# matthiasverstraete/3d_recognizer

Measured on AMD Instinct MI355X. Metric: training clouds/sec, N=40960 pts, bs=8, at 1/2/4/8 GPUs; mIoU parity, higher is better.
Workload: dtype f32 storage/accumulate, bf16x3 MFMA in the wide GEMMs

## Files before the change

3d_recognizer_amd/csrc/rows.hip:

```cpp
#include "rl_common.h"

namespace {

struct RowsParams {
    const float* src;
    long lds, src_bstride;
    float* dst;
    long ldd;
    long rows, rows_per_batch;
    int C;
    const int32_t* i32;
    const int64_t* i64;
    int shared;
    int accumulate;
    RlLazy lazy;
};

template <typename I>
__device__ __forceinline__ long src_row(const RowsParams& p, I r) {
    const I b = r / (I)p.rows_per_batch;
    const I i = r - b * (I)p.rows_per_batch;
    long j = i;
    if (p.i32) j = p.shared ? p.i32[i] : p.i32[r];
    else if (p.i64) j = p.shared ? p.i64[i] : p.i64[r];
// ... 188 lines not shown
    }
}

template <typename I>
__global__ __launch_bounds__(256) void attpool_bwd_kernel(const float* __restrict__ X, const float* __restrict__ S,
                                                          const float* __restrict__ Pout, const float* __restrict__ dP,
                                                          long P, int K, int C, float* __restrict__ dS,
                                                          float* __restrict__ dXa) {
    const long total = P * C;
    for (long e = (long)blockIdx.x * 256 + threadIdx.x; e < total; e += (long)gridDim.x * 256) {
        const long pt = (long)((I)e / (I)C);
        const int c = (int)(e - pt * C);
        const long base = pt * K * C + c;
        float m = S[base];
        for (int k = 1; k < K; ++k) m = fmaxf(m, S[base + (long)k * C]);
        float den = 0.f;
        for (int k = 0; k < K; ++k) den += expf(S[base + (long)k * C] - m);
        const float inv = 1.f / den, g = dP[e], po = Pout[e];
        for (int k = 0; k < K; ++k) {
            const long o = base + (long)k * C;
            const float a = expf(S[o] - m) * inv;
            dXa[o] = g * a;
            dS[o] = a * g * (X[o] - po);
        }
    }
}

__global__ __launch_bounds__(256) void add_act_fwd_vec_kernel(const float* __restrict__ Y1, const float* __restrict__ s1,
                                                              const float* __restrict__ b1, const float* __restrict__ Y2,
                                                              const float* __restrict__ s2, const float* __restrict__ b2,
                                                              long quads, int C, float slope, float* __restrict__ O) {
    typedef float v4f __attribute__((ext_vector_type(4)));
    const unsigned cq = (unsigned)C >> 2;
    const long stride = (long)gridDim.x * 256;
    auto one = [&](long q) {
        const int c = (int)((unsigned long)q % cq) * 4;
        const v4f y1 = *reinterpret_cast<const v4f*>(Y1 + q * 4), y2 = *reinterpret_cast<const v4f*>(Y2 + q * 4);
        const v4f a1 = *reinterpret_cast<const v4f*>(s1 + c), c1 = *reinterpret_cast<const v4f*>(b1 + c);
        const v4f a2 = *reinterpret_cast<const v4f*>(s2 + c), c2 = *reinterpret_cast<const v4f*>(b2 + c);
        const v4f z = (y1 * a1 + c1) + (y2 * a2 + c2);
        v4f o;
#pragma unroll
        for (int j = 0; j < 4; ++j) o[j] = z[j] > 0.f ? z[j] : z[j] * slope;
        *reinterpret_cast<v4f*>(O + q * 4) = o;
    };
    long q = (long)blockIdx.x * 256 + threadIdx.x;
// ... 215 lines not shown
        hipLaunchKernelGGL(attpool_fwd_kernel<int64_t>, dim3(grid_for(P * C)), dim3(256), 0, (hipStream_t)stream, X, S, (long)P, K, C, Pout);
    }
    rl_note_kernel("attpool_fwd_kernel");
    RL_LAUNCH_CHECK("rl_attpool_fwd");
    return RL_OK;
}

extern "C" int rl_attpool_bwd(const float* X, const float* S, const float* Pout, const float* dP, int64_t P, int K,
                              int C, float* dS, float* dXa, void* stream) {
    RL_REQUIRE(X && S && Pout && dP && dS && dXa && P >= 0 && K > 0 && C > 0, RL_ERR_ARGS, "rl_attpool_bwd: bad arguments");
    if (P == 0) return RL_OK;
    if (fits32(P * C) && K == 16)
        hipLaunchKernelGGL(attpool_bwd16_kernel<uint32_t>, dim3(grid_for(P * C)), dim3(256), 0, (hipStream_t)stream, X, S, Pout, dP,
                           (long)P, C, dS, dXa);
    else if (fits32(P * C))
        hipLaunchKernelGGL(attpool_bwd_kernel<uint32_t>, dim3(grid_for(P * C)), dim3(256), 0, (hipStream_t)stream, X, S, Pout, dP,
                           (long)P, K, C, dS, dXa);
    else
        hipLaunchKernelGGL(attpool_bwd_kernel<int64_t>, dim3(grid_for(P * C)), dim3(256), 0, (hipStream_t)stream, X, S, Pout, dP,
                           (long)P, K, C, dS, dXa);
    rl_note_kernel("attpool_bwd_kernel");
    RL_LAUNCH_CHECK("rl_attpool_bwd");
    return RL_OK;
}

extern "C" int rl_add_act_fwd(const float* Y1, const float* s1, const float* b1, const float* Y2, const float* s2,
                              const float* b2, int64_t rows, int C, float slope, float* O, void* stream) {
    RL_REQUIRE(Y1 && s1 && b1 && Y2 && s2 && b2 && O && rows >= 0 && C > 0, RL_ERR_ARGS, "rl_add_act_fwd: bad arguments");
    if (rows == 0) return RL_OK;
    const bool vec = C % 4 == 0 && ((((uintptr_t)Y1) | ((uintptr_t)Y2) | ((uintptr_t)O) | ((uintptr_t)s1) | ((uintptr_t)b1) |
                                      ((uintptr_t)s2) | ((uintptr_t)b2)) & 15) == 0;
    if (vec) {
        const long quads = (long)rows * (C / 4);
        hipLaunchKernelGGL(add_act_fwd_vec_kernel, dim3(grid_for((quads + 1) / 2)), dim3(256), 0, (hipStream_t)stream, Y1, s1, b1, Y2,
                           s2, b2, quads, C, slope, O);
    } else if (fits32(rows * C))
        hipLaunchKernelGGL(add_act_fwd_kernel<uint32_t>, dim3(grid_for(rows * C)), dim3(256), 0, (hipStream_t)stream, Y1, s1, b1, Y2,
                           s2, b2, (long)rows * C, C, slope, O);
    else
        hipLaunchKernelGGL(add_act_fwd_kernel<int64_t>, dim3(grid_for(rows * C)), dim3(256), 0, (hipStream_t)stream, Y1, s1, b1, Y2,
                           s2, b2, (long)rows * C, C, slope, O);
    rl_note_kernel("add_act_fwd_kernel");
    RL_LAUNCH_CHECK("rl_add_act_fwd");
    return RL_OK;
}

// ... 130 lines not shown
```

3d_recognizer_amd/randlanet/_engine.py:

```python
from typing import Dict, List, Optional

import torch

from . import _hip as H
from . import _ops as ops
from ._ops import Lazy, Rpe

BN_EPS = 1e-6
BN_MOMENTUM = 0.99
BN_PIVOT = True
BAND_SORT_MIN_POINTS = 4096


class _Tape(list):

    def __init__(self):
        super().__init__()
        self.levels: List[int] = []

    def append(self, rec) -> None:
        super().append(rec)
        self.levels.append(ops.LEVEL)

    def clear(self) -> None:
# ... 127 lines not shown
            ctx.tape.append(("linear", a, out, wname, bname, ks, ns, True))
            outs.append(out)
        return outs[0], outs[1]

    def _mlp(self, ctx, a, name: str, n_out: int, act: int = H.ACT_NONE, slope: float = 0.0, *, transposed=False,
             bn=True, a_grad=True) -> Lazy:
        return self._linear(ctx, a, f"{name}.conv.weight", f"{name}.conv.bias", n_out, transposed=transposed,
                            bn=f"{name}.batch_norm" if bn else None, act=act, slope=slope, a_grad=a_grad)

    def _pool(self, ctx, name: str, u, g: Lazy, idx: torch.Tensor, csr, n: int, d: int, n_out: int, stage: int = 0,
              next_stats: bool = False) -> Lazy:
        B, K, h = u.B, self.K, d // 2
        rows = B * n * K
        Ws = self.P[f"{name}.score_fn.0.weight"]
        if ops.pool_supported(d, K):
            if next_stats:
                res, st2, ns2 = ops.pool_fwd(u, g, idx, Ws, n, d, stage, next_stats=True)
                ctx.next_stats = (st2, ns2)
            else:
                res = ops.pool_fwd(u, g, idx, Ws, n, d, stage)
            pooled = ops.plain(res, B, n)
            ctx.tape.append(("pool_fused", name, u, g, csr, idx, pooled, n, d, stage))
            return self._mlp(ctx, pooled, f"{name}.mlp", n_out, H.ACT_RELU)
        X = torch.empty((rows, d), dtype=torch.float32, device=u.raw.device)
        ops.copy_rows_pair(((u.raw, (0, h), n * K, X, (0, h), rows, n * K), dict(lazy=u)),
                           ((g.raw, (0, h), g.bstride, X, (h, h), rows, n * K), dict(index=idx, lazy=g)))
        S = ops.gemm(ops.plain(X, B, n * K), Ws, 1, d, d, None, wsplit=getattr(ctx, "wsplit", None))
        Pt = ops.attpool_fwd(X, S, B * n, K)
        pooled = ops.plain(Pt, B, n)
        ctx.tape.append(("pool", name, u, g, csr, X, S, pooled, n, d))
        return self._mlp(ctx, pooled, f"{name}.mlp", n_out, H.ACT_RELU)

    def _virtual_bn(self, ctx: Context, vr, stage: int, bn_name: str, stats=None, nslots: int = 1) -> Lazy:
        if ctx.training and stats is None:
            stats, nslots = ops.rpe_stats(vr, stage)
        scale, shift, mean, invstd = self._fold(ctx, bn_name, stats, vr.rows, vr.h, None, nslots)
        rec = Lazy(vr.d2, vr.B, vr.n * 16, vr.n * 16, vr.h, scale, shift, H.ACT_RELU, 0.0, mean, invstd, bn_name)
        return rec

    def _lfa(self, ctx, l: int, xin: Lazy, xyz: torch.Tensor, n: int, d: int, idx, d2, csr=None) -> Lazy:
        e = f"encoder.{l}"
        B, K, h = xin.B, self.K, d // 2
        ctx.keep += [idx, d2]
        ctx.bn_defer = [] if self.sync is None else None
        f0, sc = self._mlp_pair(ctx, xin, (f"{e}.mlp1", h, H.ACT_LRELU, 0.2), (f"{e}.shortcut", 2 * d, H.ACT_NONE, 0.0))
        if ops.virtual_rpe_supported(d, K, B * n, n):
# ... 4 lines not shown
            ops.bn_finalize_flush(ctx.bn_defer)
            q1 = self._pool(ctx, f"{e}.pool1", vr, f0, idx, csr, n, d, h, stage=1, next_stats=ctx.training)
            vr.bn2 = self._virtual_bn(ctx, vr, 2, f"{e}.mlp_rpe2.batch_norm", *getattr(ctx, "next_stats", (None, 1)))
            ctx.next_stats = (None, 1)
            ops.bn_finalize_flush(ctx.bn_defer)
            ctx.bn_defer = None
            q2 = self._pool(ctx, f"{e}.pool2", vr, q1, idx, csr, n, d, d, stage=2)
        else:
            rpe = Rpe(xyz, idx, d2, B, n, K)
            if h <= 128:
                rpe = ops.rpe_build(rpe)
            u1 = self._mlp(ctx, rpe, f"{e}.mlp_rpe1", h, H.ACT_RELU, a_grad=False)
            ops.bn_finalize_flush(ctx.bn_defer)
            q1 = self._pool(ctx, f"{e}.pool1", u1, f0, idx, csr, n, d, h)
            u2 = self._mlp(ctx, u1, f"{e}.mlp_rpe2", h, H.ACT_RELU)
            ops.bn_finalize_flush(ctx.bn_defer)
            ctx.bn_defer = None
            q2 = self._pool(ctx, f"{e}.pool2", u2, q1, idx, csr, n, d, d)
        m2 = self._mlp(ctx, q2, f"{e}.mlp2", 2 * d)
        O = ops.plain(ops.add_act_fwd(m2, sc, 0.01), B, n)
        ctx.tape.append(("add_act", m2, sc, O))
        return O

    def _wide_weight_uses(self, training: bool):
        uses = []
        for name, W in self.P.items():
            if not name.endswith(("conv.weight", "score_fn.0.weight")) or W.dim() < 2:
                continue
            a, b = int(W.shape[0]), int(W.shape[1])
            if max(a, b) <= 64:
                if name.endswith(".mlp1.conv.weight") and b % 32 == 0 and b > 64:
                    sc = self.P.get(name.replace(".mlp1.", ".shortcut."))
                    if sc is not None and int(sc.shape[0]) > 64:
                        uses.append((W.view(a, b), 1, b, b, a, True))
                continue
            transposed = name.startswith("decoder.")
            K, N = (a, b) if transposed else (b, a)
            ks, ns = (N, 1) if transposed else (1, K)
            W2 = W.view(a, b)
            uses.append((W2, ks, ns, K, N))
            if training:
                uses.append((W2, ns, ks, N, K))
        return uses

    def min_points(self) -> int:
        L = len(self.layers)
        return max(self.K * self.dec ** (L - 1), 2 * self.dec ** L)

    def prepare(self, inp: torch.Tensor, perm: torch.Tensor, training: bool) -> "Prep":
        B, N, cin = inp.shape
        assert cin == 3 + self.F and inp.dtype == torch.float32 and inp.is_cuda and inp.is_contiguous()
        assert perm.dtype == torch.int64 and perm.numel() == N and perm.is_cuda
# ... 36 lines not shown
        prep.xyz4, prep.searches = xyz4, searches
        prep.csrs = ops.csr_build([(searches[i][0], tasks[i][0]) for i in range(2 * L)]) if training else [None] * (2 * L)
        return prep

    def forward(self, inp: torch.Tensor, perm: torch.Tensor, training: bool, dropout_p: float = 0.5,
                keep_mask: Optional[torch.Tensor] = None, logits_out: Optional[torch.Tensor] = None,
                prep: Optional["Prep"] = None, head: Optional[ops.Head] = None):
        B, N, cin = inp.shape
        assert cin == 3 + self.F and inp.dtype == torch.float32 and inp.is_cuda and inp.is_contiguous()
        assert perm.dtype == torch.int64 and perm.numel() == N and perm.is_cuda
        assert N >= self.min_points()
        dev = inp.device
        ctx = Context()
        ctx.training, ctx.B, ctx.N, ctx.perm = training, B, N, perm
        L, dec = len(self.layers), self.dec
        ctx.eval_folds = None
        ctx.eval_sig = tuple(ops.virtual_rpe_supported(d, self.K, B * (N // dec ** l), N // dec ** l) for l, d in enumerate(self.layers))
        if not training:
            self._eval_spec_build = {}
            spec = self._eval_specs.get(ctx.eval_sig)
            if spec is not None and self.sync is None:
                ctx.eval_folds = self._eval_folds(spec)

        ctx.wsplit = ops.split_weights(self._wide_weight_uses(training))
        if prep is None:
            prep = self.prepare(inp, perm, training)
        perm = prep.perm
        ctx.perm = perm
        assert prep.B == B and prep.N == N and prep.training >= training
        inp_p, xyz, searches, csrs = prep.inp_p, prep.xyz, prep.searches, prep.csrs
        ctx.keep += [inp_p, xyz]
        if prep.xyz4 is not None:
            ctx.keep.append(prep.xyz4)
        ctx.xyz4 = prep.xyz4

        a0 = ops.plain(inp_p, B, N)
        if cin == 3 and prep.xyz4 is not None:
            a0 = Lazy(prep.xyz4.view(B * N, 4), B, N, N, 3)
        x = self._linear(ctx, a0, "fc_start.weight", "fc_start.bias", 8, bn="bn_start.0",
                         act=H.ACT_LRELU, slope=0.2, a_grad=False)
        skips: List[Lazy] = []
        ratio = 1
        for l, d in enumerate(self.layers):
            n_l = N // ratio
            ops.LEVEL = l
            x = self._lfa(ctx, l, x.prefix(n_l), xyz, n_l, d, *searches[l], csr=csrs[l])
            ops.LEVEL = -1
# ... 68 lines not shown
    def backward(self, ctx: Context, dlogits: torch.Tensor, grads: Dict[str, torch.Tensor]) -> None:
        if not ctx.training:
            raise H.HipKernelError("backward is implemented for training-mode forwards (batch statistics)")
        B, N = ctx.B, ctx.N
        fused_head = bool(ctx.tape) and ctx.tape[-1][0] == "head"
        if not fused_head:
            assert dlogits.shape == (B, self.C, N) and dlogits.is_cuda
            dlogits = dlogits.contiguous().float()
            ctx.grads[id(ctx.logits_perm.raw)] = [ops.logits_permute_grad(dlogits, ctx.perm), True]
        ctx.bn_pre = {}
        ctx.bn_done = set()
        ctx.fin_queue, ctx.rpe_after = [], []
        ctx.pending = []
        ctx.wbatch = []
        for rec, lvl in zip(reversed(ctx.tape), reversed(ctx.tape.levels)):
            ops.LEVEL = lvl
            kind = rec[0]
            if kind != "linear":
                self._flush_rpe(ctx)
            if kind == "linear":
                self._bwd_linear(ctx, grads, *rec[1:])
            elif kind == "pool":
                self._bwd_pool(ctx, grads, *rec[1:])
            elif kind == "pool_fused":
                _, name, u, g, csr, idx, pooled, n, d, stage = rec
                if stage:
                    self._bwd_pool_virtual(ctx, grads, name, u, g, csr, idx, pooled, n, d, stage)
                    continue
                GP, init = self._gbuf(ctx, pooled)
                assert init
                gu, gg = self._gbuf(ctx, u), self._gbuf(ctx, g)
                DG = ops.pool_bwd(u, g, idx, self.P[f"{name}.score_fn.0.weight"], n, d, GP, gu[0], gu[1],
                                  grads[f"{name}.score_fn.0.weight"], pending=ctx.pending, batch=ctx.wbatch)
                gu[1] = True
                ops.segment_sum_rows(DG, (0, d // 2), n * self.K, csr, gg[0], g.bstride, accumulate=gg[1])
                gg[1] = True
            elif kind == "add_act":
                _, m2, sc, O = rec
                G, init = self._gbuf(ctx, O)
                assert init
                if ops.resid_bn_supported(m2, sc):
                    g2 = ops.resid_bn_backward(G, O.raw, 0.01, m2, sc, grads[f"{m2.bn}.weight"], grads[f"{m2.bn}.bias"],
                                               grads[f"{sc.bn}.weight"], grads[f"{sc.bn}.bias"], sync=self.sync)
                    ctx.bn_done.update((id(m2.raw), id(sc.raw)))
                else:
                    ops.add_act_bwd(G, O.raw, 0.01)
# ... 125 lines not shown

    def _bwd_pool(self, ctx, grads, name, u: Lazy, g: Lazy, csr, X, S, pooled: Lazy, n, d):
        B, K, h = u.B, self.K, d // 2
        rows = B * n * K
        GP, init = self._gbuf(ctx, pooled)
        assert init
        dS, dX = ops.attpool_bwd(X, S, pooled.raw, GP, B * n, K)
        Ws = self.P[f"{name}.score_fn.0.weight"]
        ops.wgrad(ops.plain(X, B, n * K), dS, n * K, d, grads[f"{name}.score_fn.0.weight"], 1, d, None, pending=ctx.pending,
                  batch=ctx.wbatch)
        gu = self._gbuf(ctx, u)
        gg = self._gbuf(ctx, g)
        if d <= 64:
            ops.gemm(ops.plain(dS, B, n * K), Ws, d, 1, d, None, out=dX, out_bstride=n * K, accumulate=True,
                     wsplit=getattr(ctx, "wsplit", None))
            ops.copy_rows(dX, (0, h), n * K, gu[0], (0, h), rows, n * K, accumulate=gu[1])
            ops.segment_sum_rows(dX, (h, h), n * K, csr, gg[0], g.bstride, accumulate=gg[1])
        else:
            DG = torch.empty((rows, h), dtype=torch.float32, device=dX.device)
            ops.gemm(ops.plain(dS, B, n * K), Ws, d, 1, d, None, out=gu[0], out_bstride=n * K, accumulate=gu[1],
                     addend=dX, out2=DG, split_col=h, wsplit=getattr(ctx, "wsplit", None))
            ops.segment_sum_rows(DG, (0, h), n * K, csr, gg[0], g.bstride, accumulate=gg[1])
        gu[1] = gg[1] = True
```

3d_recognizer_amd/randlanet/_hip.py:

```python
import ctypes as C
import os
from typing import Optional

import torch

_LIB: Optional[C.CDLL] = None
_LIB_PATH = os.path.join(os.path.dirname(os.path.dirname(os.path.abspath(__file__))), "csrc",
                         "librandla_hip.so")
_LIB_PATH = os.environ.get("RL_HIP_LIB", _LIB_PATH)

ABI_VERSION = 110
MAX_SLOTS = 1024
KNN_MAX_K = 64
ACT_NONE, ACT_RELU, ACT_LRELU = 0, 1, 2

ERR_ARGS, ERR_FEW_SUPPORT, ERR_LAUNCH, ERR_UNSUPPORTED = -1, -2, -3, -4


class HipKernelError(RuntimeError):
    pass


class GemmDesc(C.Structure):
    _fields_ = [
# ... 133 lines not shown
    _fields_ = [
        ("stats", C.c_void_p), ("count", C.c_int64), ("gamma", C.c_void_p), ("beta", C.c_void_p),
        ("running_mean", C.c_void_p), ("running_var", C.c_void_p), ("num_batches_tracked", C.c_void_p),
        ("scale", C.c_void_p), ("shift", C.c_void_p), ("save_mean", C.c_void_p), ("save_invstd", C.c_void_p),
        ("folded_bias", C.c_void_p), ("nslots", C.c_int32), ("C", C.c_int32), ("training", C.c_int32),
        ("momentum", C.c_float), ("eps", C.c_float), ("pivoted", C.c_int32), ("pivot", C.c_void_p),
    ]


class BnBwdFinalizeItem(C.Structure):
    _fields_ = [
        ("stats", C.c_void_p), ("count", C.c_int64), ("dgamma", C.c_void_p), ("dbeta", C.c_void_p), ("coef", C.c_void_p),
        ("nslots", C.c_int32), ("C", C.c_int32),
    ]


class SegsumDesc(C.Structure):
    _fields_ = [
        ("src", C.c_void_p), ("lds", C.c_int64), ("src_bstride", C.c_int64),
        ("dst", C.c_void_p), ("ldd", C.c_int64), ("dst_bstride", C.c_int64),
        ("offsets", C.c_void_p), ("entries", C.c_void_p), ("entries_per_cloud", C.c_int64),
        ("B", C.c_int32), ("n_dst", C.c_int32), ("C", C.c_int32), ("accumulate", C.c_int32),
        ("src_bf16", C.c_int32),
    ]


class RowsDesc(C.Structure):
    _fields_ = [
        ("src", C.c_void_p), ("lds", C.c_int64), ("src_bstride", C.c_int64),
        ("dst", C.c_void_p), ("ldd", C.c_int64),
        ("rows", C.c_int64), ("rows_per_batch", C.c_int64),
        ("C", C.c_int32),
        ("index32", C.c_void_p), ("index64", C.c_void_p),
        ("index_shared", C.c_int32), ("accumulate", C.c_int32), ("act", C.c_int32),
        ("slope", C.c_float),
        ("scale", C.c_void_p), ("shift", C.c_void_p),
    ]


_vp, _i, _l, _f = C.c_void_p, C.c_int, C.c_int64, C.c_float
_SIGNATURES = {
    "rl_last_error": (C.c_char_p, []),
    "rl_last_kernel": (C.c_char_p, []),
    "rl_version": (_i, []),
    "rl_spin_us": (_i, [_i, _vp]),
    "rl_launch_count": (_l, []),
# ... 43 lines not shown
    "rl_resid_bn_bwd_apply": (_i, [C.POINTER(ResidBnBwdDesc), _vp]),
    "rl_resid_bn_bwd_fused_supported": (_i, [_l, _i]),
    "rl_resid_bn_bwd_fused": (_i, [C.POINTER(ResidBnBwdDesc), _vp, _vp, _vp, _vp, _vp]),
    "rl_copy_rows": (_i, [C.POINTER(RowsDesc), _vp]),
    "rl_copy_rows_pair": (_i, [C.POINTER(RowsDesc), C.POINTER(RowsDesc), _vp]),
    "rl_scatter_add_rows": (_i, [C.POINTER(RowsDesc), _vp]),
    "rl_csr_workspace_bytes": (_l, [C.POINTER(CsrTask), _i, _i]),
    "rl_csr_build": (_i, [C.POINTER(CsrTask), _i, _i, _vp, _l, _vp]),
    "rl_segment_sum_rows": (_i, [C.POINTER(SegsumDesc), _vp]),
    "rl_pool_supported": (_i, [_i, _i]),
    "rl_pool_slab_floats": (_l, [_l, _i]),
    "rl_pool_bwd_slots": (_i, [_l, _i]),
    "rl_pool_bwd_grid": (_i, [_l, _i, _i]),
    "rl_pool_fwd_slots": (_i, [_l, _i]),
    "rl_pool_fwd": (_i, [C.POINTER(PoolDesc), _vp]),
    "rl_rpe_stats_slots": (_i, [_l]),
    "rl_rpe_stats": (_i, [C.POINTER(PoolDesc), _vp, _vp]),
    "rl_rpe_bn_reduce": (_i, [C.POINTER(PoolDesc), _vp, _vp, _vp]),
    "rl_rpe_wgrad_slab_floats": (_l, [_l, _i, _i]),
    "rl_rpe_wgrad": (_i, [C.POINTER(PoolDesc), _vp, _vp, _vp, _l, _vp, _vp]),
    "rl_pool_bwd": (_i, [C.POINTER(PoolDesc), _vp]),
    "rl_attpool_fwd": (_i, [_vp, _vp, _l, _i, _i, _vp, _vp]),
    "rl_attpool_bwd": (_i, [_vp, _vp, _vp, _vp, _l, _i, _i, _vp, _vp, _vp]),
    "rl_add_act_fwd": (_i, [_vp, _vp, _vp, _vp, _vp, _vp, _l, _i, _f, _vp, _vp]),
    "rl_add_act_bwd": (_i, [_vp, _vp, _l, _i, _f, _vp]),
    "rl_rpe_build": (_i, [_vp, _l, _vp, _vp, _i, _i, _i, _vp, _vp]),
    "rl_rpe_build_dist": (_i, [_vp, _l, _vp, _vp, _i, _i, _i, _vp, _vp]),
    "rl_batch_assemble": (_i, [_vp, _i, _i, _i, _vp, _vp, _vp, _vp, _vp, _vp]),
    "rl_batch_assemble_scratch_doubles": (_l, [_i, _i]),
    "rl_batch_assemble_flag_u32": (_l, [_i, _i, _i]),
    "rl_batch_draw": (_i, [_vp, _i, _i, C.c_uint64, _vp, _vp, _vp]),
    "rl_scale_mask": (_i, [_vp, _vp, _f, _l, _vp]),
    "rl_dropout_tick": (_i, [_vp, _vp, _vp]),
    "rl_dropout_fwd": (_i, [_vp, _vp, _vp, _i, _f, _vp, _l, _l, _i, _vp, C.c_uint64, _f, _vp]),
    "rl_dropout_bwd": (_i, [_vp, _l, _l, _i, _vp, C.c_uint64, _f, _vp]),
    "rl_upsample_cf": (_i, [_vp, _vp, _vp, _i, _i, _i, _i, _i, _i, _vp, _vp]),
    "rl_logits_unpermute": (_i, [_vp, _vp, _i, _i, _i, _vp, _vp]),
    "rl_logits_permute_grad": (_i, [_vp, _vp, _i, _i, _i, _vp, _vp]),
    "rl_logits_unpermute_b": (_i, [_vp, _vp, C.c_int64, _i, _i, _i, _vp, _vp]),
    "rl_logits_permute_grad_b": (_i, [_vp, _vp, C.c_int64, _i, _i, _i, _vp, _vp]),
    "rl_band_sort_workspace_bytes": (C.c_int64, [_i, _i, _vp, _i]),
    "rl_band_sort": (_i, [_vp, C.c_int64, _vp, _i, _i, _vp, _i, _vp, _vp, C.c_int64, _vp]),
    "rl_loss_work_doubles": (_l, [_l, _i]),
    "rl_loss_forward": (_i, [_vp, _vp, _i, _i, _i, _i, _f, _f, _i, _vp, _vp, _vp]),
    "rl_loss_backward": (_i, [_vp, _vp, _i, _i, _i, _i, _f, _f, _i, _vp, _f, _vp, _vp]),
    "rl_loss_partials": (_i, [_vp, _vp, _i, _i, _i, _i, _f, _vp, _vp]),
# ... 69 lines not shown
```

3d_recognizer_amd/randlanet/_ops.py:

```python
import ctypes as C
import os
from dataclasses import dataclass
from typing import Optional, Tuple

import torch

from . import _hip as H

F32 = torch.float32
BF16 = torch.bfloat16

_STORAGE = os.environ.get("RL_STORAGE", "f32")


def set_storage(mode: str) -> None:
    global _STORAGE
    if mode not in ("f32", "bf16"):
        raise ValueError(f"storage must be 'f32' or 'bf16', got {mode!r}")
    if mode == "bf16" and get_wide_gemm() == "fp32":
        raise H.HipKernelError("bf16 storage needs the bf16x3 / bf16 arithmetic mode (RL_WIDE_GEMM)")
    _STORAGE = mode


def get_storage() -> str:
# ... 27 lines not shown
        assert n <= self.n
        return Lazy(self.raw, self.B, n, self.bstride, self.C, self.scale, self.shift, self.act,
                    self.slope, self.mean, self.invstd, self.bn)


def plain(t: torch.Tensor, B: int, n: int) -> Lazy:
    assert t.dim() == 2 and t.shape[0] == B * n and t.is_contiguous()
    return Lazy(t, B, n, n, t.shape[1])


def _dev_check(*ts):
    cur = H.current_device()
    for t in ts:
        if t is None:
            continue
        if not t.is_cuda:
            raise H.HipKernelError("HIP kernels need device tensors")
        if t.get_device() != cur:
            raise H.HipKernelError(
                f"tensor on cuda:{t.get_device()} but the current device is cuda:{cur}: run under "
                "`with torch.cuda.device(tensor.device)` (launches use the current device's stream)")
        if not t.is_contiguous():
            raise H.HipKernelError("HIP kernels need contiguous tensors")


def _st():
    return H.stream_ptr()


class KernelTimer:

    def __init__(self):
        self.records = []

    def summary(self):
        torch.cuda.synchronize()
        agg = {}
        for cat, key, nbytes, flops, e0, e1, _kern, _lvl in self.records:
            a = agg.setdefault((cat, key), dict(category=cat, shape=key, launches=0, ms=0.0, bytes=0, flops=0))
            a["launches"] += 1
            a["ms"] += e0.elapsed_time(e1)
            a["bytes"] += nbytes
            a["flops"] += flops
        return sorted(agg.values(), key=lambda a: -a["ms"])


# ... 162 lines not shown

def weight_strides(W: torch.Tensor, transposed: bool, K: int, N: int) -> Tuple[int, int]:
    if transposed:
        assert W.shape[0] == K and W.shape[1] == N, (tuple(W.shape), K, N)
        return N, 1
    assert W.shape[0] == N and W.shape[1] == K, (tuple(W.shape), K, N)
    return 1, K




def split_weights(entries) -> dict:
    out_map = {}
    if get_wide_gemm() == "fp32" or not entries:
        return out_map
    entries = [e[:5] for e in entries if e[3] % 8 == 0 and (e[4] > 64 or e[3] > 64 or len(e) > 5)]
    if not entries:
        return out_map
    total = sum(2 * K * N + 8 for _, _, _, K, N in entries)
    buf = torch.empty(total, dtype=torch.bfloat16, device=entries[0][0].device)
    arr = (H.WsplitItem * len(entries))()
    off = 0
    for it, (W, ks, ns, K, N) in zip(arr, entries):
        _dev_check(W)
        assert W.dtype == F32 and W.numel() == K * N
        out = buf[off:off + 2 * K * N]
        it.W, it.w_ks, it.w_ns, it.K, it.N, it.out = W.data_ptr(), ks, ns, K, N, out.data_ptr()
        out_map[(W.data_ptr(), ks, ns, K, N)] = out
        off += (2 * K * N + 7) // 8 * 8
    with _rec("split_weights", (len(entries),), 6 * sum(K * N for _, _, _, K, N in entries), 0):
        H.check(H.lib().rl_split_weights(arr, len(entries), _st()), "rl_split_weights")
    return out_map


def gemm_stat_slots(M: int, N: int, K: int) -> int:
    return int(H.lib().rl_gemm_stat_slots(M, N, K))


def gemm(a, W: torch.Tensor, w_ks: int, w_ns: int, N: int, bias: Optional[torch.Tensor] = None, *,
         out: Optional[torch.Tensor] = None, out_bstride: Optional[int] = None,
         accumulate: bool = False, stats: Optional[torch.Tensor] = None,
         addend: Optional[torch.Tensor] = None, out2: Optional[torch.Tensor] = None,
         out2_index: Optional[torch.Tensor] = None, out2_bstride: int = 0, split_col: int = 0,
         wsplit: Optional[dict] = None, pivot: Optional[tuple] = None, bnb: Optional[Lazy] = None):
    d = H.GemmDesc()
    M, K = _fill_a(d, a)
    assert isinstance(a, Rpe) or a.raw.dtype == F32, "rl_gemm reads fp32 rows"
    rows_per_batch = a.n * a.K if isinstance(a, Rpe) else a.n
    _dev_check(W, bias, out, stats)
    assert W.dtype == F32 and W.numel() == K * N
    if out is None:
        out = torch.empty((M, N), dtype=F32, device=W.device)
        out_bstride = rows_per_batch
    else:
        assert out.dtype == F32 and out.dim() == 2 and out.shape[1] >= (split_col if out2 is not None else N)
        out_bstride = rows_per_batch if out_bstride is None else out_bstride
        assert out.shape[0] >= (d.B - 1) * out_bstride + rows_per_batch, "Y rows out of range"
    if bias is not None:
        assert bias.numel() == N
    if stats is not None:
        assert stats.dtype == torch.float64 and stats.numel() >= gemm_stat_slots(M, N, K) * 2 * N
    d.N, d.W, d.w_ks, d.w_ns, d.bias = N, W.data_ptr(), w_ks, w_ns, H.ptr(bias)
    planes = wsplit.get((W.data_ptr(), w_ks, w_ns, K, N)) if wsplit else None
    if planes is not None:
        d.W_split = planes.data_ptr()
    d.Y, d.ldy, d.y_bstride, d.accumulate = out.data_ptr(), out.shape[1], out_bstride, int(accumulate)
    d.stats = H.ptr(stats)
    if pivot is not None:
        assert stats is not None and pivot[0].numel() == N and (pivot[1] is None or pivot[1].numel() == N)
        _dev_check(*pivot)
        d.stats_pivot_mean, d.stats_pivot_bias = pivot[0].data_ptr(), H.ptr(pivot[1])
    if addend is not None or out2 is not None:
# ... 62 lines not shown
    return outs[0], outs[1]


_SLAB = {}


def _slab(device, floats: int) -> torch.Tensor:
    key = (device, torch.cuda.current_stream(device).cuda_stream)
    buf = _SLAB.get(key)
    if buf is None or buf.numel() < floats:
        buf = torch.empty(max(floats, 1 << 20), dtype=F32, device=device)
        _SLAB[key] = buf
    return buf


WGRAD_BATCH_BYTES = 3 << 30


def wgrad(a, dY: torch.Tensor, dy_bstride: int, N: int, dW: torch.Tensor, w_ks: int, w_ns: int,
          dbias: Optional[torch.Tensor] = None, pending: Optional[list] = None, batch: Optional[list] = None) -> None:
    d = H.WgradDesc()
    M, K = _fill_a(d, a)
    rows_per_batch = a.n * a.K if isinstance(a, Rpe) else a.n
    _dev_check(dY, dW, dbias)
    rows_bf16 = dY.dtype == BF16
    assert dY.dtype in (F32, BF16) and dY.dim() == 2 and dY.shape[1] >= N
    assert isinstance(a, Rpe) or a.raw.dtype == dY.dtype, "A and dY must share their storage type"
    d.rows_bf16 = int(rows_bf16)
    assert dY.shape[0] >= (d.B - 1) * dy_bstride + rows_per_batch
    assert dW.numel() == K * N and (dbias is None or dbias.numel() == N)
    floats = H.lib().rl_wgrad_slab_floats(M, N, K)
    slab = _slab(dY.device, floats) if pending is None else torch.empty(floats, dtype=F32, device=dY.device)
    d.N, d.dY, d.lddy, d.dy_bstride = N, dY.data_ptr(), dY.shape[1], dy_bstride
    d.dW, d.w_ks, d.w_ns, d.dbias = dW.data_ptr(), w_ks, w_ns, H.ptr(dbias)
    d.slab, d.slab_floats = slab.data_ptr(), slab.numel()
    d.defer_reduce = 0 if pending is None else 1
    es = 2 if rows_bf16 else 4
    nbytes, flops = es * (M * (K if not isinstance(a, Rpe) else 6) + M * N) + 4 * K * N, 2 * M * K * N
    kind = H.lib().rl_wgrad_batchable(C.byref(d)) if (batch is not None and pending is not None) else 0
    if kind:
        batch.append((d, nbytes, flops, a, dY, slab, kind))
        if sum(b[1] for b in batch) > WGRAD_BATCH_BYTES:
            wgrad_batch_flush(batch)
    else:
        with _rec("wgrad_rpe" if isinstance(a, Rpe) else "wgrad", (M, K, N), nbytes, flops):
            H.check(H.lib().rl_wgrad(C.byref(d), _st()), "rl_wgrad")
    if pending is not None:
# ... 535 lines not shown

def attpool_fwd(X: torch.Tensor, S: torch.Tensor, P: int, K: int) -> torch.Tensor:
    _dev_check(X, S)
    Cc = X.shape[1]
    assert X.shape == S.shape == (P * K, Cc)
    out = torch.empty((P, Cc), dtype=F32, device=X.device)
    with _rec("attpool_fwd", (P, K, Cc), 4 * (2 * P * K * Cc + P * Cc), 0):
        H.check(H.lib().rl_attpool_fwd(X.data_ptr(), S.data_ptr(), P, K, Cc, out.data_ptr(), _st()), "rl_attpool_fwd")
    return out


def attpool_bwd(X, S, Pout, dP, P: int, K: int):
    _dev_check(X, S, Pout, dP)
    Cc = X.shape[1]
    assert X.shape == S.shape == (P * K, Cc) and Pout.shape == dP.shape == (P, Cc)
    dS = torch.empty_like(S)
    dXa = torch.empty_like(X)
    with _rec("attpool_bwd", (P, K, Cc), 4 * (4 * P * K * Cc + 2 * P * Cc), 0):
        H.check(H.lib().rl_attpool_bwd(X.data_ptr(), S.data_ptr(), Pout.data_ptr(), dP.data_ptr(), P, K, Cc,
                                       dS.data_ptr(), dXa.data_ptr(), _st()), "rl_attpool_bwd")
    return dS, dXa


def add_act_fwd(y1: Lazy, y2: Lazy, slope: float) -> torch.Tensor:
    assert y1.rows == y2.rows and y1.C == y2.C and y1.bstride == y1.n and y2.bstride == y2.n
    out = torch.empty((y1.rows, y1.C), dtype=F32, device=y1.raw.device)
    with _rec("add_act", (y1.rows, y1.C), 12 * y1.rows * y1.C, 0):
        H.check(H.lib().rl_add_act_fwd(y1.raw.data_ptr(), y1.scale.data_ptr(), y1.shift.data_ptr(), y2.raw.data_ptr(),
                                       y2.scale.data_ptr(), y2.shift.data_ptr(), y1.rows, y1.C, slope, out.data_ptr(),
                                       _st()), "rl_add_act_fwd")
    return out


def add_act_bwd(G: torch.Tensor, O: torch.Tensor, slope: float) -> None:
    assert G.shape == O.shape and G.is_contiguous() and O.is_contiguous()
    with _rec("add_act", (G.shape[0], G.shape[1]), 12 * G.numel(), 0):
        H.check(H.lib().rl_add_act_bwd(G.data_ptr(), O.data_ptr(), G.shape[0], G.shape[1], slope, _st()), "rl_add_act_bwd")


def scale_mask(x: torch.Tensor, mask: torch.Tensor, scale: float) -> None:
    _dev_check(x, mask)
    assert mask.dtype == torch.uint8 and mask.numel() == x.numel() and x.dtype == F32
    H.check(H.lib().rl_scale_mask(x.data_ptr(), mask.data_ptr(), scale, x.numel(), _st()), "rl_scale_mask")


def dropout_tick(counter: torch.Tensor) -> torch.Tensor:
# ... 290 lines not shown
```

include/rl_randlanet.h:

```cpp
#ifndef RL_RANDLANET_H
#define RL_RANDLANET_H

#include <stdint.h>

#ifdef __cplusplus
extern "C" {
#endif

#define RL_VERSION 110

#define RL_OK 0
#define RL_ERR_ARGS (-1)
#define RL_ERR_FEW_SUPPORT (-2)
#define RL_ERR_LAUNCH (-3)
#define RL_ERR_UNSUPPORTED (-4)

#define RL_MAX_SLOTS 1024
#define RL_KNN_MAX_K 64

const char* rl_last_error(void);
const char* rl_last_kernel(void);
int rl_version(void);
int64_t rl_launch_count(void);
int rl_spin_us(int us, void* stream);
// ... 243 lines not shown
int64_t rl_csr_workspace_bytes(const rl_csr_task* tasks, int ntasks, int B);
int rl_csr_build(const rl_csr_task* tasks, int ntasks, int B, void* workspace, int64_t workspace_bytes,
                 void* stream);

typedef struct rl_segsum_desc {
    const float* src;
    int64_t lds, src_bstride;
    float* dst;
    int64_t ldd, dst_bstride;
    const int32_t* offsets;
    const int32_t* entries;
    int64_t entries_per_cloud;
    int32_t B, n_dst, C;
    int32_t accumulate;
    int32_t src_bf16;
} rl_segsum_desc;

int rl_segment_sum_rows(const rl_segsum_desc* d, void* stream);

int rl_attpool_fwd(const float* X, const float* S, int64_t P, int K, int C, float* Pout,
                   void* stream);
int rl_attpool_bwd(const float* X, const float* S, const float* Pout, const float* dP, int64_t P,
                   int K, int C, float* dS, float* dXa, void* stream);

typedef struct rl_pool_desc {
    const float* U;
    const float* u_scale;
    const float* u_shift;
    int32_t u_act;
    float u_slope;
    const float* G;
    int64_t g_bstride;
    const float* g_scale;
    const float* g_shift;
    int32_t g_act;
    float g_slope;
    const int32_t* idx;
    const float* W;
    int64_t points;
    int32_t n, d, nbr_k;
    float* Pout;
    const float* dP;
    float* GU;
    int32_t gu_accumulate;
    float* DG;
    float* dW;
// ... 175 lines not shown
```

Baseline: 1282.

## Split attentive-pooling score GEMM into per-point and per-neighbor halves

The attentive-pooling score GEMM over the concatenated [u, gathered g] rows is split by linearity into u·Ws[:, :h] over all point-neighbor rows plus g·Ws[:, h:] computed once per source point and gathered by index. New fused kernels add the gathered T to Su, apply the softmax-weighted pooling and its backward directly from u and g with their lazy BN/activation, and skip the materialized X concat buffer. This removes a large gather-copy and halves the K-expanded GEMM width, at the cost of an extra gathered read of T, a segment-sum for dT and more GEMM/wgrad launches. It is only enabled for large, non-fused pooling layers.

Measured after the change: 1259. 1.8% lower.

```diff
diff --git a/3d_recognizer_amd/csrc/rows.hip b/3d_recognizer_amd/csrc/rows.hip
--- a/3d_recognizer_amd/csrc/rows.hip
+++ b/3d_recognizer_amd/csrc/rows.hip
@@ -234,6 +234,174 @@
             const float a = expf(S[o] - m) * inv;
             dXa[o] = g * a;
             dS[o] = a * g * (X[o] - po);
+        }
+    }
+}
+
+struct SplitParams {
+    const float* u; long ldu; RlLazy ul;
+    const float* g; long ldg, g_bstride; RlLazy gl;
+    const int32_t* idx;
+    const float* Su; const float* T;
+    long P; int n, K, C;
+    float* Pout; const float* dP;
+    float* dS; float* dXa_u; float* dXa_g;
+};
+
+template <int V> struct SplitVec { typedef float type __attribute__((ext_vector_type(V))); };
+template <> struct SplitVec<1> { typedef float type; };
+
+template <int V>
+__device__ __forceinline__ typename SplitVec<V>::type split_exp(typename SplitVec<V>::type z) {
+    if constexpr (V == 1) return expf(z);
+    else {
+        typename SplitVec<V>::type r;
+#pragma unroll
+        for (int j = 0; j < V; ++j) r[j] = expf(z[j]);
+        return r;
+    }
+}
+
+template <int V>
+struct SplitSrc {
+    typedef typename SplitVec<V>::type vec;
+    const float* x; long ld; bool lo;
+    vec sc, sh; float es; bool lazy;
+    __device__ __forceinline__ SplitSrc(const SplitParams& p, long pt, long b, int c) {
+        const int h = p.C / 2;
+        lo = c < h;
+        const RlLazy& l = lo ? p.ul : p.gl;
+        const int cc = lo ? c : c - h;
+        x = lo ? p.u + pt * p.K * p.ldu + cc : p.g + b * p.g_bstride * p.ldg + cc;
+        ld = lo ? p.ldu : p.ldg;
+        lazy = l.scale != nullptr;
+        es = (!lazy || l.act == RL_ACT_NONE) ? 1.f : (l.act == RL_ACT_RELU ? 0.f : l.slope);
+        if (lazy) {
+            sc = *reinterpret_cast<const vec*>(l.scale + cc);
+            sh = *reinterpret_cast<const vec*>(l.shift + cc);
+        } else {
+            sc = 1.f; sh = 0.f;
+        }
+    }
+    __device__ __forceinline__ long row(int k, int j) const { return (lo ? (long)k : (long)j) * ld; }
+    __device__ __forceinline__ vec act(vec v) const {
+        if (!lazy) return v;
+        const vec z = v * sc + sh;
+        if constexpr (V == 1) return fmaxf(z, z * es);
+        else return __builtin_elementwise_max(z, z * es);
+    }
+};
+
+template <int V>
+__device__ __forceinline__ typename SplitVec<V>::type split_max(typename SplitVec<V>::type a, typename SplitVec<V>::type b) {
+    if constexpr (V == 1) return fmaxf(a, b);
+    else return __builtin_elementwise_max(a, b);
+}
+
+template <int V, bool BWD>
+__global__ __launch_bounds__(256) void attpool_split16_kernel(const SplitParams p) {
+    typedef typename SplitVec<V>::type vec;
+    const unsigned cpr = (unsigned)(p.C / V);
+    const long total = p.P * cpr;
+    const int h = p.C / 2;
+    for (long e = (long)blockIdx.x * 256 + threadIdx.x; e < total; e += (long)gridDim.x * 256) {
+        const unsigned pt = (unsigned)e / cpr;
+        const int c = (int)((unsigned)e - pt * cpr) * V;
+        const unsigned b = pt / (unsigned)p.n;
+        int j[16];
+        {
+            const int4* ip = reinterpret_cast<const int4*>(p.idx + (long)pt * 16);
+#pragma unroll
+            for (int q = 0; q < 4; ++q) {
+                const int4 t = ip[q];
+                j[4 * q] = t.x; j[4 * q + 1] = t.y; j[4 * q + 2] = t.z; j[4 * q + 3] = t.w;
+            }
+        }
+        const SplitSrc<V> src(p, pt, b, c);
+        const float* su = p.Su + (long)pt * 16 * p.C + c;
+        const float* tt = p.T + (long)b * p.n * p.C + c;
+        vec sv[16], xv[16];
+#pragma unroll
+        for (int k = 0; k < 16; ++k) sv[k] = *reinterpret_cast<const vec*>(su + (long)k * p.C);
+#pragma unroll
+        for (int k = 0; k < 16; ++k) sv[k] += *reinterpret_cast<const vec*>(tt + (long)j[k] * p.C);
+#pragma unroll
+        for (int k = 0; k < 16; ++k) xv[k] = src.act(*reinterpret_cast<const vec*>(src.x + src.row(k, j[k])));
+        vec m = sv[0];
+#pragma unroll
+        for (int k = 1; k < 16; ++k) m = split_max<V>(m, sv[k]);
+        const long o = (long)pt * p.C + c;
+        if constexpr (!BWD) {
+            vec den = 0.f, num = 0.f;
+#pragma unroll
+            for (int k = 0; k < 16; ++k) {
+                const vec w = split_exp<V>(sv[k] - m);
+                den += w;
+                num += w * xv[k];
+            }
+            *reinterpret_cast<vec*>(p.Pout + o) = num / den;
+        } else {
+            const vec gp = *reinterpret_cast<const vec*>(p.dP + o), po = *reinterpret_cast<const vec*>(p.Pout + o);
+            vec den = 0.f;
+#pragma unroll
+            for (int k = 0; k < 16; ++k) {
+                sv[k] = split_exp<V>(sv[k] - m);
+                den += sv[k];
+            }
+            const vec inv = 1.f / den;
+            float* dxa = (src.lo ? p.dXa_u + c : p.dXa_g + (c - h)) + (long)pt * 16 * h;
+            float* ds = p.dS + (long)pt * 16 * p.C + c;
+#pragma unroll
+            for (int k = 0; k < 16; ++k) {
+                const vec a = sv[k] * inv;
+                *reinterpret_cast<vec*>(dxa + (long)k * h) = gp * a;
+                *reinterpret_cast<vec*>(ds + (long)k * p.C) = a * gp * (xv[k] - po);
+            }
+        }
+    }
+}
+
+template <int V, bool BWD>
+__global__ __launch_bounds__(256) void attpool_split_kernel(const SplitParams p) {
+    typedef typename SplitVec<V>::type vec;
+    const unsigned cpr = (unsigned)(p.C / V);
+    const long total = p.P * cpr;
+    const int h = p.C / 2, K = p.K;
+    for (long e = (long)blockIdx.x * 256 + threadIdx.x; e < total; e += (long)gridDim.x * 256) {
+        const unsigned pt = (unsigned)e / cpr;
+        const int c = (int)((unsigned)e - pt * cpr) * V;
+        const unsigned b = pt / (unsigned)p.n;
+        const int32_t* j = p.idx + (long)pt * K;
+        const SplitSrc<V> src(p, pt, b, c);
+        const float* su = p.Su + (long)pt * K * p.C + c;
+        const float* tt = p.T + (long)b * p.n * p.C + c;
+        auto score = [&](int k) -> vec {
+            return *reinterpret_cast<const vec*>(su + (long)k * p.C) + *reinterpret_cast<const vec*>(tt + (long)j[k] * p.C);
+        };
+        vec m = score(0);
+        for (int k = 1; k < K; ++k) m = split_max<V>(m, score(k));
+        const long o = (long)pt * p.C + c;
+        if constexpr (!BWD) {
+            vec den = 0.f, num = 0.f;
+            for (int k = 0; k < K; ++k) {
+                const vec w = split_exp<V>(score(k) - m);
+                den += w;
+                num += w * src.act(*reinterpret_cast<const vec*>(src.x + src.row(k, j[k])));
+            }
+            *reinterpret_cast<vec*>(p.Pout + o) = num / den;
+        } else {
+            vec den = 0.f;
+            for (int k = 0; k < K; ++k) den += split_exp<V>(score(k) - m);
+            const vec inv = 1.f / den;
+            const vec gp = *reinterpret_cast<const vec*>(p.dP + o), po = *reinterpret_cast<const vec*>(p.Pout + o);
+            float* dxa = (src.lo ? p.dXa_u + c : p.dXa_g + (c - h)) + (long)pt * K * h;
+            float* ds = p.dS + (long)pt * K * p.C + c;
+            for (int k = 0; k < K; ++k) {
+                const vec a = split_exp<V>(score(k) - m) * inv;
+                const vec x = src.act(*reinterpret_cast<const vec*>(src.x + src.row(k, j[k])));
+                *reinterpret_cast<vec*>(dxa + (long)k * h) = gp * a;
+                *reinterpret_cast<vec*>(ds + (long)k * p.C) = a * gp * (x - po);
+            }
         }
     }
 }
@@ -495,6 +663,55 @@
     rl_note_kernel("attpool_bwd_kernel");
     RL_LAUNCH_CHECK("rl_attpool_bwd");
     return RL_OK;
+}
+
+static int attpool_split_launch(const rl_attpool_split_desc* d, bool bwd, void* stream, const char* who) {
+    RL_REQUIRE(d != nullptr, RL_ERR_ARGS, "%s: null descriptor", who);
+    RL_REQUIRE(d->U && d->G && d->idx && d->Su && d->T && d->Pout, RL_ERR_ARGS, "%s: missing operand", who);
+    RL_REQUIRE(d->points >= 0 && d->n > 0 && d->points % d->n == 0 && d->nbr_k > 0 && d->d >= 2 && d->d % 2 == 0, RL_ERR_ARGS,
+               "%s: bad sizes points=%ld n=%d K=%d d=%d", who, (long)d->points, d->n, d->nbr_k, d->d);
+    const int h = d->d / 2;
+    RL_REQUIRE(d->ldu >= h && d->ldg >= h && d->g_bstride >= d->n, RL_ERR_ARGS, "%s: bad row strides", who);
+    RL_REQUIRE((d->u_scale == nullptr) == (d->u_shift == nullptr) && (d->g_scale == nullptr) == (d->g_shift == nullptr), RL_ERR_ARGS,
+               "%s: scale/shift must come together", who);
+    RL_REQUIRE(!bwd || (d->dP && d->dS && d->dXa_u && d->dXa_g), RL_ERR_ARGS, "%s: missing gradient operand", who);
+    RL_REQUIRE(d->points * d->d < (1l << 32), RL_ERR_ARGS, "%s: too many elements", who);
+    SplitParams p{};
+    p.u = d->U; p.ldu = d->ldu; p.ul.scale = d->u_scale; p.ul.shift = d->u_shift; p.ul.act = d->u_act; p.ul.slope = d->u_slope;
+    p.g = d->G; p.ldg = d->ldg; p.g_bstride = d->g_bstride;
+    p.gl.scale = d->g_scale; p.gl.shift = d->g_shift; p.gl.act = d->g_act; p.gl.slope = d->g_slope;
+    p.idx = d->idx; p.Su = d->Su; p.T = d->T; p.P = d->points; p.n = d->n; p.K = d->nbr_k; p.C = d->d;
+    p.Pout = d->Pout; p.dP = d->dP; p.dS = d->dS; p.dXa_u = d->dXa_u; p.dXa_g = d->dXa_g;
+    if (d->points == 0) return RL_OK;
+    uintptr_t al = (uintptr_t)d->U | (uintptr_t)d->G | (uintptr_t)d->Su | (uintptr_t)d->T | (uintptr_t)d->Pout | (uintptr_t)d->u_scale |
+                   (uintptr_t)d->u_shift | (uintptr_t)d->g_scale | (uintptr_t)d->g_shift | (uintptr_t)d->idx;
+    if (bwd) al |= (uintptr_t)d->dP | (uintptr_t)d->dS | (uintptr_t)d->dXa_u | (uintptr_t)d->dXa_g;
+    const bool quads = h % 4 == 0 && d->ldu % 4 == 0 && d->ldg % 4 == 0 && (al & 15) == 0;
+    const bool k16 = d->nbr_k == 16;
+    RL_REQUIRE(!k16 || ((uintptr_t)d->idx & 15) == 0, RL_ERR_ARGS, "%s: idx must be 16-byte aligned", who);
+    const dim3 grid(grid_for(d->points * (d->d / (quads && !k16 ? 4 : 1)))), block(256);
+    hipStream_t st = (hipStream_t)stream;
+    if (k16) {
+        if (bwd) hipLaunchKernelGGL((attpool_split16_kernel<1, true>), grid, block, 0, st, p);
+        else     hipLaunchKernelGGL((attpool_split16_kernel<1, false>), grid, block, 0, st, p);
+    } else if (quads) {
+        if (bwd) hipLaunchKernelGGL((attpool_split_kernel<4, true>), grid, block, 0, st, p);
+        else     hipLaunchKernelGGL((attpool_split_kernel<4, false>), grid, block, 0, st, p);
+    } else {
+        if (bwd) hipLaunchKernelGGL((attpool_split_kernel<1, true>), grid, block, 0, st, p);
+        else     hipLaunchKernelGGL((attpool_split_kernel<1, false>), grid, block, 0, st, p);
+    }
+    rl_note_kernel(bwd ? "attpool_split_bwd_kernel" : "attpool_split_fwd_kernel");
+    RL_LAUNCH_CHECK(who);
+    return RL_OK;
+}
+
+extern "C" int rl_attpool_split_fwd(const rl_attpool_split_desc* d, void* stream) {
+    return attpool_split_launch(d, false, stream, "rl_attpool_split_fwd");
+}
+
+extern "C" int rl_attpool_split_bwd(const rl_attpool_split_desc* d, void* stream) {
+    return attpool_split_launch(d, true, stream, "rl_attpool_split_bwd");
 }
 
 extern "C" int rl_add_act_fwd(const float* Y1, const float* s1, const float* b1, const float* Y2, const float* s2,
diff --git a/3d_recognizer_amd/randlanet/_engine.py b/3d_recognizer_amd/randlanet/_engine.py
--- a/3d_recognizer_amd/randlanet/_engine.py
+++ b/3d_recognizer_amd/randlanet/_engine.py
@@ -173,6 +173,14 @@
             pooled = ops.plain(res, B, n)
             ctx.tape.append(("pool_fused", name, u, g, csr, idx, pooled, n, d, stage))
             return self._mlp(ctx, pooled, f"{name}.mlp", n_out, H.ACT_RELU)
+        if self._split_score(B, n, d):
+            ws = getattr(ctx, "wsplit", None)
+            T = ops.gemm(g.prefix(n), Ws[:, h:], 1, d, d, None, wsplit=ws)
+            Su = ops.gemm(u, Ws[:, :h], 1, d, d, None, wsplit=ws)
+            Pt = ops.attpool_split_fwd(u, g, idx, Su, T, n, d)
+            pooled = ops.plain(Pt, B, n)
+            ctx.tape.append(("pool_split", name, u, g, csr, idx, Su, T, pooled, n, d))
+            return self._mlp(ctx, pooled, f"{name}.mlp", n_out, H.ACT_RELU)
         X = torch.empty((rows, d), dtype=torch.float32, device=u.raw.device)
         ops.copy_rows_pair(((u.raw, (0, h), n * K, X, (0, h), rows, n * K), dict(lazy=u)),
                            ((g.raw, (0, h), g.bstride, X, (h, h), rows, n * K), dict(index=idx, lazy=g)))
@@ -223,12 +231,24 @@
         ctx.tape.append(("add_act", m2, sc, O))
         return O
 
-    def _wide_weight_uses(self, training: bool):
+    def _split_score(self, B: int, n: int, d: int) -> bool:
+        return (not ops.NO_SPLIT_SCORE and not ops.pool_supported(d, self.K)
+                and 4 * B * n * self.K * d >= ops.SPLIT_SCORE_MIN_BYTES)
+
+    def _wide_weight_uses(self, training: bool, B: int = 0, N: int = 0):
         uses = []
         for name, W in self.P.items():
             if not name.endswith(("conv.weight", "score_fn.0.weight")) or W.dim() < 2:
                 continue
             a, b = int(W.shape[0]), int(W.shape[1])
+            if name.endswith("score_fn.0.weight") and name.startswith("encoder.") and B > 0 and \
+                    self._split_score(B, N // self.dec ** int(name.split(".")[1]), a):
+                h = b // 2
+                for Wb in (W[:, :h], W[:, h:]):
+                    uses.append((Wb, 1, b, h, a))
+                    if training:
+                        uses.append((Wb, b, 1, a, h))
+                continue
             if max(a, b) <= 64:
                 if name.endswith(".mlp1.conv.weight") and b % 32 == 0 and b > 64:
                     sc = self.P.get(name.replace(".mlp1.", ".shortcut."))
@@ -311,7 +331,7 @@
             if spec is not None and self.sync is None:
                 ctx.eval_folds = self._eval_folds(spec)
 
-        ctx.wsplit = ops.split_weights(self._wide_weight_uses(training))
+        ctx.wsplit = ops.split_weights(self._wide_weight_uses(training, B, N))
         if prep is None:
             prep = self.prepare(inp, perm, training)
         perm = prep.perm
@@ -426,6 +446,8 @@
                 self._bwd_linear(ctx, grads, *rec[1:])
             elif kind == "pool":
                 self._bwd_pool(ctx, grads, *rec[1:])
+            elif kind == "pool_split":
+                self._bwd_pool_split(ctx, grads, *rec[1:])
             elif kind == "pool_fused":
                 _, name, u, g, csr, idx, pooled, n, d, stage = rec
                 if stage:
@@ -597,3 +619,26 @@
                      addend=dX, out2=DG, split_col=h, wsplit=getattr(ctx, "wsplit", None))
             ops.segment_sum_rows(DG, (0, h), n * K, csr, gg[0], g.bstride, accumulate=gg[1])
         gu[1] = gg[1] = True
+
+    def _bwd_pool_split(self, ctx, grads, name, u: Lazy, g: Lazy, csr, idx, Su, T, pooled: Lazy, n, d):
+        B, K, h = u.B, self.K, d // 2
+        rows = B * n * K
+        GP, init = self._gbuf(ctx, pooled)
+        assert init
+        dS, dXa_u, dXa_g = ops.attpool_split_bwd(u, g, idx, Su, T, n, d, pooled.raw, GP)
+        Ws, dWs = self.P[f"{name}.score_fn.0.weight"], grads[f"{name}.score_fn.0.weight"]
+        ws = getattr(ctx, "wsplit", None)
+        gu, gg = self._gbuf(ctx, u), self._gbuf(ctx, g)
+        ops.segment_sum_rows(dXa_g, (0, h), n * K, csr, gg[0], g.bstride, accumulate=gg[1])
+        dT = torch.empty((B * n, d), dtype=torch.float32, device=dS.device)
+        ops.segment_sum_rows(dS, (0, d), n * K, csr, dT, n)
+        ops.gemm(ops.plain(dT, B, n), Ws[:, h:], d, 1, h, None, out=gg[0], out_bstride=g.bstride, accumulate=True, wsplit=ws)
+        ops.wgrad(g.prefix(n), dT, n, d, dWs[:, h:], 1, d, None, pending=ctx.pending, batch=ctx.wbatch)
+        ops.wgrad(u, dS, n * K, d, dWs[:, :h], 1, d, None, pending=ctx.pending, batch=ctx.wbatch)
+        if d <= 64:
+            ops.gemm(ops.plain(dS, B, n * K), Ws[:, :h], d, 1, h, None, out=dXa_u, out_bstride=n * K, accumulate=True, wsplit=ws)
+            ops.copy_rows(dXa_u, (0, h), n * K, gu[0], (0, h), rows, n * K, accumulate=gu[1])
+        else:
+            ops.gemm(ops.plain(dS, B, n * K), Ws[:, :h], d, 1, h, None, out=gu[0], out_bstride=n * K, accumulate=gu[1],
+                     addend=dXa_u, wsplit=ws)
+        gu[1] = gg[1] = True
diff --git a/3d_recognizer_amd/randlanet/_hip.py b/3d_recognizer_amd/randlanet/_hip.py
--- a/3d_recognizer_amd/randlanet/_hip.py
+++ b/3d_recognizer_amd/randlanet/_hip.py
@@ -179,6 +179,18 @@
         ("offsets", C.c_void_p), ("entries", C.c_void_p), ("entries_per_cloud", C.c_int64),
         ("B", C.c_int32), ("n_dst", C.c_int32), ("C", C.c_int32), ("accumulate", C.c_int32),
         ("src_bf16", C.c_int32),
+    ]
+
+
+class AttpoolSplitDesc(C.Structure):
+    _fields_ = [
+        ("U", C.c_void_p), ("ldu", C.c_int64), ("u_scale", C.c_void_p), ("u_shift", C.c_void_p), ("u_act", C.c_int32),
+        ("u_slope", C.c_float),
+        ("G", C.c_void_p), ("ldg", C.c_int64), ("g_bstride", C.c_int64), ("g_scale", C.c_void_p), ("g_shift", C.c_void_p),
+        ("g_act", C.c_int32), ("g_slope", C.c_float),
+        ("idx", C.c_void_p), ("Su", C.c_void_p), ("T", C.c_void_p),
+        ("points", C.c_int64), ("n", C.c_int32), ("d", C.c_int32), ("nbr_k", C.c_int32),
+        ("Pout", C.c_void_p), ("dP", C.c_void_p), ("dS", C.c_void_p), ("dXa_u", C.c_void_p), ("dXa_g", C.c_void_p),
     ]
 
 
@@ -268,6 +280,8 @@
     "rl_pool_bwd": (_i, [C.POINTER(PoolDesc), _vp]),
     "rl_attpool_fwd": (_i, [_vp, _vp, _l, _i, _i, _vp, _vp]),
     "rl_attpool_bwd": (_i, [_vp, _vp, _vp, _vp, _l, _i, _i, _vp, _vp, _vp]),
+    "rl_attpool_split_fwd": (_i, [C.POINTER(AttpoolSplitDesc), _vp]),
+    "rl_attpool_split_bwd": (_i, [C.POINTER(AttpoolSplitDesc), _vp]),
     "rl_add_act_fwd": (_i, [_vp, _vp, _vp, _vp, _vp, _vp, _l, _i, _f, _vp, _vp]),
     "rl_add_act_bwd": (_i, [_vp, _vp, _l, _i, _f, _vp]),
     "rl_rpe_build": (_i, [_vp, _l, _vp, _vp, _i, _i, _i, _vp, _vp]),
diff --git a/3d_recognizer_amd/randlanet/_ops.py b/3d_recognizer_amd/randlanet/_ops.py
--- a/3d_recognizer_amd/randlanet/_ops.py
+++ b/3d_recognizer_amd/randlanet/_ops.py
@@ -73,6 +73,14 @@
                 "`with torch.cuda.device(tensor.device)` (launches use the current device's stream)")
         if not t.is_contiguous():
             raise H.HipKernelError("HIP kernels need contiguous tensors")
+
+
+def _w_check(W: torch.Tensor) -> None:
+    if W.is_contiguous():
+        _dev_check(W)
+        return
+    assert W.dim() == 2 and W.stride(1) == 1 and W.stride(0) >= W.shape[1], "weight view must be a column block"
+    _dev_check(W[:1])
 
 
 def _st():
@@ -281,7 +289,7 @@
     arr = (H.WsplitItem * len(entries))()
     off = 0
     for it, (W, ks, ns, K, N) in zip(arr, entries):
-        _dev_check(W)
+        _w_check(W)
         assert W.dtype == F32 and W.numel() == K * N
         out = buf[off:off + 2 * K * N]
         it.W, it.w_ks, it.w_ns, it.K, it.N, it.out = W.data_ptr(), ks, ns, K, N, out.data_ptr()
@@ -306,7 +314,8 @@
     M, K = _fill_a(d, a)
     assert isinstance(a, Rpe) or a.raw.dtype == F32, "rl_gemm reads fp32 rows"
     rows_per_batch = a.n * a.K if isinstance(a, Rpe) else a.n
-    _dev_check(W, bias, out, stats)
+    _dev_check(bias, out, stats)
+    _w_check(W)
     assert W.dtype == F32 and W.numel() == K * N
     if out is None:
         out = torch.empty((M, N), dtype=F32, device=W.device)
@@ -415,7 +424,8 @@
     d = H.WgradDesc()
     M, K = _fill_a(d, a)
     rows_per_batch = a.n * a.K if isinstance(a, Rpe) else a.n
-    _dev_check(dY, dW, dbias)
+    _dev_check(dY, dbias)
+    _w_check(dW)
     rows_bf16 = dY.dtype == BF16
     assert dY.dtype in (F32, BF16) and dY.dim() == 2 and dY.shape[1] >= N
     assert isinstance(a, Rpe) or a.raw.dtype == dY.dtype, "A and dY must share their storage type"
@@ -997,6 +1007,54 @@
     return dS, dXa
 
 
+NO_SPLIT_SCORE = False
+SPLIT_SCORE_MIN_BYTES = 32 << 20
+
+
+def _attpool_split_desc(u: Lazy, g: Lazy, idx: torch.Tensor, Su: torch.Tensor, T: torch.Tensor, n: int, d: int) -> "H.AttpoolSplitDesc":
+    B, h = u.B, d // 2
+    K = idx.shape[-1]
+    _dev_check(u.raw, u.scale, u.shift, g.raw, g.scale, g.shift, idx, Su, T)
+    assert u.raw.dtype == F32 and g.raw.dtype == F32 and Su.dtype == F32 and T.dtype == F32 and idx.dtype == torch.int32
+    assert u.C == h and g.C == h and u.n == n * K and u.bstride == n * K and u.raw.shape[0] >= B * n * K and g.n >= n
+    assert g.raw.shape[0] >= (B - 1) * g.bstride + n and idx.numel() == B * n * K
+    assert Su.shape == (B * n * K, d) and T.shape == (B * n, d)
+    pd = H.AttpoolSplitDesc()
+    pd.U, pd.ldu, pd.G, pd.ldg, pd.g_bstride = u.raw.data_ptr(), u.raw.shape[1], g.raw.data_ptr(), g.raw.shape[1], g.bstride
+    if u.scale is not None:
+        pd.u_scale, pd.u_shift, pd.u_act, pd.u_slope = u.scale.data_ptr(), u.shift.data_ptr(), u.act, u.slope
+    if g.scale is not None:
+        pd.g_scale, pd.g_shift, pd.g_act, pd.g_slope = g.scale.data_ptr(), g.shift.data_ptr(), g.act, g.slope
+    pd.idx, pd.Su, pd.T = idx.data_ptr(), Su.data_ptr(), T.data_ptr()
+    pd.points, pd.n, pd.d, pd.nbr_k = B * n, n, d, K
+    return pd
+
+
+def attpool_split_fwd(u: Lazy, g: Lazy, idx: torch.Tensor, Su: torch.Tensor, T: torch.Tensor, n: int, d: int) -> torch.Tensor:
+    pd = _attpool_split_desc(u, g, idx, Su, T, n, d)
+    P, K = u.B * n, idx.shape[-1]
+    out = torch.empty((P, d), dtype=F32, device=Su.device)
+    pd.Pout = out.data_ptr()
+    with _rec("attpool_split_fwd", (P, K, d), 4 * (P * K * (d + d // 2 + 1) + 2 * P * K * d // 2 + P * d), 0):
+        H.check(H.lib().rl_attpool_split_fwd(C.byref(pd), _st()), "rl_attpool_split_fwd")
+    return out
+
+
+def attpool_split_bwd(u: Lazy, g: Lazy, idx: torch.Tensor, Su: torch.Tensor, T: torch.Tensor, n: int, d: int,
+                      Pout: torch.Tensor, dP: torch.Tensor):
+    pd = _attpool_split_desc(u, g, idx, Su, T, n, d)
+    P, K, h = u.B * n, idx.shape[-1], d // 2
+    _dev_check(Pout, dP)
+    assert Pout.shape == dP.shape == (P, d) and Pout.dtype == F32 and dP.dtype == F32
+    dS = torch.empty((P * K, d), dtype=F32, device=Su.device)
+    dXa_u = torch.empty((P * K, h), dtype=F32, device=Su.device)
+    dXa_g = torch.empty((P * K, h), dtype=F32, device=Su.device)
+    pd.Pout, pd.dP, pd.dS, pd.dXa_u, pd.dXa_g = Pout.data_ptr(), dP.data_ptr(), dS.data_ptr(), dXa_u.data_ptr(), dXa_g.data_ptr()
+    with _rec("attpool_split_bwd", (P, K, d), 4 * (P * K * (d + d // 2 + 1) + 2 * P * K * d // 2 + 2 * P * K * d + 2 * P * d), 0):
+        H.check(H.lib().rl_attpool_split_bwd(C.byref(pd), _st()), "rl_attpool_split_bwd")
+    return dS, dXa_u, dXa_g
+
+
 def add_act_fwd(y1: Lazy, y2: Lazy, slope: float) -> torch.Tensor:
     assert y1.rows == y2.rows and y1.C == y2.C and y1.bstride == y1.n and y2.bstride == y2.n
     out = torch.empty((y1.rows, y1.C), dtype=F32, device=y1.raw.device)
diff --git a/include/rl_randlanet.h b/include/rl_randlanet.h
--- a/include/rl_randlanet.h
+++ b/include/rl_randlanet.h
@@ -289,6 +289,34 @@
                    void* stream);
 int rl_attpool_bwd(const float* X, const float* S, const float* Pout, const float* dP, int64_t P,
                    int K, int C, float* dS, float* dXa, void* stream);
+
+typedef struct rl_attpool_split_desc {
+    const float* U;
+    int64_t ldu;
+    const float* u_scale;
+    const float* u_shift;
+    int32_t u_act;
+    float u_slope;
+    const float* G;
+    int64_t ldg, g_bstride;
+    const float* g_scale;
+    const float* g_shift;
+    int32_t g_act;
+    float g_slope;
+    const int32_t* idx;
+    const float* Su;
+    const float* T;
+    int64_t points;
+    int32_t n, d, nbr_k;
+    float* Pout;
+    const float* dP;
+    float* dS;
+    float* dXa_u;
+    float* dXa_g;
+} rl_attpool_split_desc;
+
+int rl_attpool_split_fwd(const rl_attpool_split_desc* d, void* stream);
+int rl_attpool_split_bwd(const rl_attpool_split_desc* d, void* stream);
 
 typedef struct rl_pool_desc {
     const float* U;
```
